# ethz-asl/reinmav-gym

Hardware: AMD Instinct MI355X
Metric: env-steps/sec (batched quadrotor3d-v0) (higher is better)
Workload: dtype f32; 1 GPU; BASELINE configs[1] (C2): quadrotor3d-v0, 65536 envs/GPU, random actions in-kernel, auto-reset; 1 step = 1 fused 64-env-step rollout launch, trajectory written to a ring of 6 buffer sets; config_id=C2, kind=quad3d, actions=random, envs_per_gpu=65536, envs_total=65536, env_steps_per_launch_per_env=64, mode=rollout, trajectory_layout=soa, trajectory_ring=6, tune=, parallelism=single GPU, finished_episodes=189717026, gathered_envs_with_a_finished_episode=65536

## Files before the change

### reinmav-gym_amd/csrc/rmav_abi.hip

```cpp
#include <cmath>
#include <cstdarg>
#include <cstdio>
#include <cstdint>
#include <cstdlib>
#include <cstring>
#include <ctime>
#include <new>

#include "rmav_handle.hpp"
#include "rmav_core_kernels.hpp"

using namespace rmav;

namespace {

thread_local char g_err[768] = "";

}

int rmav_fail(int code, const char *fmt, ...) {
    va_list ap;
    va_start(ap, fmt);
    vsnprintf(g_err, sizeof(g_err), fmt, ap);
    va_end(ap);
// ... 147 lines not shown
constexpr int64_t kEnvsPerCuSlot = 16384;
constexpr bool kSliceByDefault = false;

template <int K, int MODE, int ST>
int launch_rollout_kms(rmav_handle h, const RolloutArgs &a_in) {
    RolloutArgs a = a_in;
    take_armed_exchange(h, a, 64, publishes_start(MODE));
    const KindParams<K> kp = kind_params<K>(h);
    static_assert(!is_policy(MODE), "the policy-in-kernel rollouts are launched from rmav_policy_abi.hip");
    const size_t lds = (ST == ST_AOS_LDS) ? sizeof(float) * AosTile<Dims<K>::NS>::WORDS * (block_size(h) / 64) : 0;
    if constexpr (is_split(MODE)) {
        constexpr size_t lds_per_pair = sizeof(float) * split_words_per_pair<K, MODE>();
        const int forced = h->tune[RMAV_TUNE_SPLIT_GROUP];
        constexpr int g_max = split_pairs_max<K, MODE>();
        const int64_t count = a.slice_count ? (int64_t)a.slice_count : h->n;
        constexpr bool latency_bound = (K == QUAD2D || K == QUAD2D_SL) || MODE == ACT_CONTROLLER_SPLIT;
        const bool one_pair = latency_bound && (count <= 98304 || K == QUAD2D);
        int g = (forced >= 1 && forced <= g_max) ? forced : one_pair ? 1 : (int)((count + kEnvsPerCuSlot - 1) / kEnvsPerCuSlot);
        if (g < 1) g = 1;
        if (g > g_max) g = g_max;
        const int64_t per_wg = 64 * g;
        if (!(a.flags & F_AOS) && (int64_t)a.n_steps * Dims<K>::NS * a.pitch < ((int64_t)1 << 30)) a.flags |= F_LEAN;
        const dim3 grid((unsigned)((count + per_wg - 1) / per_wg)), block(128 * g);
        bool launched = false;
        if constexpr (ST == ST_WRITE_THROUGH) {
            if ((a.flags & (F_AOS | F_TRACK | F_AUTO_RESET)) == (F_TRACK | F_AUTO_RESET)) {
                hipLaunchKernelGGL((k_rollout<K, MODE, ST, true>), grid, block, lds_per_pair * g, h->stream, a, kp.p, kp.pc);
                launched = true;
            }
        }
        if (!launched) hipLaunchKernelGGL((k_rollout<K, MODE, ST>), grid, block, lds_per_pair * g, h->stream, a, kp.p, kp.pc);
    } else if (h->range_mask) {
        if constexpr (K != REINMAV && (MODE == ACT_BUFFER || MODE == ACT_RANDOM || MODE == ACT_CONTROLLER)) {
            if (int rc = rmav_launch_ranged_rollout(h, MODE, ST, a)) return rc;
        } else {
            return rmav_fail(RMAV_ERR_INVALID, "no ranged kernel for action mode %d", MODE);
        }
    } else {
        if (h->time_limit > 0) {
            if constexpr (K != REINMAV && (MODE == ACT_BUFFER || MODE == ACT_RANDOM || MODE == ACT_CONTROLLER)) {
                const int64_t count = a.slice_count ? (int64_t)a.slice_count : h->n;
                const dim3 grid((unsigned)((count + block_size(h) - 1) / block_size(h)));
                hipLaunchKernelGGL((k_rollout_tl<K, MODE, ST>), grid, dim3(block_size(h)), lds, h->stream, a, kp.p, kp.pc, tl_args(h));
            } else {
                return rmav_fail(RMAV_ERR_INVALID, "no time-limited kernel for action mode %d", MODE);
            }
        } else {
            hipLaunchKernelGGL((k_rollout<K, MODE, ST>), grid_for(h), dim3(block_size(h)), lds, h->stream, a, kp.p, kp.pc);
        }
    }
    return check_rollout_launch(h, a);
}

bool use_split(rmav_handle h, const RolloutArgs &a, int action_mode, int *slices, bool random_actions) {
// ... 1051 lines not shown
```

### reinmav-gym_amd/csrc/rmav_kernels.hpp

```cpp
#pragma once

#include "rmav_math.hpp"
#include "rmav_policy.hpp"
#include "rmav_policy_mfma.hpp"
#include "rmav_policy_mfma32.hpp"

namespace rmav {

enum : int { ACT_BUFFER = 0, ACT_RANDOM = 1, ACT_CONTROLLER = 2, ACT_POLICY = 3, ACT_POLICY_BF16 = 4,
              ACT_RANDOM_SPLIT = 5, ACT_CONTROLLER_SPLIT = 6,
              ACT_BUFFER_CTRL = 7,
              ACT_POLICY_F32M = 8,
              ACT_BUFFER_SPLIT = 9,
              ACT_POLICY_F16 = 10,
              ACT_POLICY_F16_SHARED = 11 };
constexpr bool is_mfma_policy(int mode) { return mode == ACT_POLICY_BF16 || mode == ACT_POLICY_F32M; }
constexpr bool is_policy(int mode) { return mode == ACT_POLICY || is_mfma_policy(mode); }
constexpr bool is_split(int mode) { return mode == ACT_RANDOM_SPLIT || mode == ACT_CONTROLLER_SPLIT || mode == ACT_BUFFER_SPLIT; }
constexpr bool split_feeds_actions(int mode) { return mode == ACT_RANDOM_SPLIT; }
constexpr bool split_self_fetch(int mode) { return mode == ACT_BUFFER_SPLIT; }
constexpr bool is_buffer(int mode) { return mode == ACT_BUFFER || mode == ACT_BUFFER_CTRL; }
constexpr bool publishes_start(int mode) { return mode != ACT_CONTROLLER_SPLIT; }
#ifndef RMAV_SPLIT_CHUNK
#define RMAV_SPLIT_CHUNK 1
// ... 205 lines not shown
#endif
typedef uint32_t u32x4_t __attribute__((ext_vector_type(4)));
template <int AUX>
__device__ __forceinline__ void buf_st4_aux(rsrc_t r, uint32_t voff, uint32_t soff, float4 v) {
    u32x4_t d;
    d[0] = __builtin_bit_cast(uint32_t, v.x);
    d[1] = __builtin_bit_cast(uint32_t, v.y);
    d[2] = __builtin_bit_cast(uint32_t, v.z);
    d[3] = __builtin_bit_cast(uint32_t, v.w);
    __builtin_amdgcn_raw_buffer_store_b128(d, r, voff, soff, AUX);
}
template <int AUX, int C>
__device__ __forceinline__ void wide_cols(const float *tile, rsrc_t r, uint32_t wave_off, uint32_t col, uint32_t lane) {
    const uint32_t cg = lane >> 4, eq = lane & 15u;
#pragma unroll
    for (int j = 0; 4 * j < C; ++j) {
        if (4 * j + 3 < C || 4 * j + (int)cg < C) {
            const float4 v = *reinterpret_cast<const float4 *>(tile + (4 * j + cg) * 64u + 4u * eq);
            buf_st4_aux<AUX>(r, wave_off + 16u * eq + cg * col, (uint32_t)(4 * j) * col, v);
        }
    }
}

template <int K, int MODE, int ST = ST_DEFAULT, bool FIXED = false>
__global__ __launch_bounds__((rollout_threads_max<K, MODE>())) void k_rollout(const RolloutArgs a, const typename Env<K>::P p_shared,
                                                    const ParamsT<double> pc_shared) {
    constexpr bool TL = false, BOOT = false, NORM = false, DR = false;
    [[maybe_unused]] const RangeArgs dr{};
    [[maybe_unused]] const ActRuleArgs ar{};
    [[maybe_unused]] const TimeLimitArgs tl{};
    [[maybe_unused]] const BootArgs bt{};
    [[maybe_unused]] const NormArgs nm{};
#include "rmav_rollout_body.inc"
}
template <int K, int MODE, int ST = ST_DEFAULT>
__global__ __launch_bounds__((rollout_threads_max<K, MODE>())) void k_rollout_tl(const RolloutArgs a, const typename Env<K>::P p_shared,
                                                       const ParamsT<double> pc_shared, const TimeLimitArgs tl) {
    constexpr bool TL = true, FIXED = false, BOOT = false, NORM = false, DR = false;
    [[maybe_unused]] const RangeArgs dr{};
    [[maybe_unused]] const ActRuleArgs ar{};
    [[maybe_unused]] const BootArgs bt{};
    [[maybe_unused]] const NormArgs nm{};
    static_assert(!is_split(MODE) && K != REINMAV, "time-limited launches run the one-wavefront kernels");
#include "rmav_rollout_body.inc"
}
template <int K, int MODE, int ST = ST_DEFAULT>
__global__ __launch_bounds__((rollout_threads_max<K, MODE>())) void k_rollout_boot(const RolloutArgs a, const typename Env<K>::P p_shared,
                                                         const ParamsT<double> pc_shared, const TimeLimitArgs tl, const BootArgs bt) {
    constexpr bool TL = true, FIXED = false, BOOT = true, NORM = false, DR = false;
    [[maybe_unused]] const RangeArgs dr{};
    [[maybe_unused]] const ActRuleArgs ar{};
    [[maybe_unused]] const NormArgs nm{};
    static_assert(MODE == ACT_POLICY_F32M && K != REINMAV, "the one-wavefront actor of time-limited handles");
#include "rmav_rollout_body.inc"
}
template <int K, bool BOOT>
__global__ __launch_bounds__((rollout_threads_max<K, ACT_POLICY_F32M>())) void k_rollout_nrm(const RolloutArgs a, const typename Env<K>::P p_shared,
// ... 398 lines not shown
```

### reinmav-gym_amd/csrc/rmav_rollout_body.inc

```
    constexpr int NS = Dims<K>::NS, NA = Dims<K>::NA;
    constexpr int AUX = StoreAux<ST>::value;
    constexpr bool SPLIT = is_split(MODE), DRAWS = split_feeds_actions(MODE);
    [[maybe_unused]] constexpr int CH = SplitTile<NS, NA, DRAWS>::CH;
    const uint32_t split_g = SPLIT ? (blockDim.x >> 7) : 1u;
    const bool upper_half = SPLIT && (uint32_t)__builtin_amdgcn_readfirstlane(threadIdx.x >> 6) >= split_g;
    const bool split_helper = upper_half;
    const uint32_t split_local = threadIdx.x - (upper_half ? 64u * split_g : 0u);
    const uint32_t gi = a.slice_first + (SPLIT ? blockIdx.x * (64u * split_g) + split_local : blockIdx.x * blockDim.x + threadIdx.x);
    const uint32_t slice_end = a.slice_count ? a.slice_first + a.slice_count : (uint32_t)a.n;
    [[maybe_unused]] float *lds_p = lds_w;
    if constexpr (SPLIT)
        lds_p = lds_w + (uint32_t)__builtin_amdgcn_readfirstlane(split_local >> 6) * SplitTile<NS, NA, DRAWS>::WORDS;
    const int64_t n = a.n;
    constexpr bool HALF = (MODE == ACT_POLICY_F32M);
    const uint32_t ge = HALF ? ((gi >> 6) << 5) + (gi & 31u) : gi;
    const bool valid = ge < slice_end;
    const uint32_t li = ((is_mfma_policy(MODE) || SPLIT) && !valid) ? slice_end - 1u : ge;
    const uint32_t col = (uint32_t)n * 4u;
    const int64_t tn = a.pitch;
    const uint32_t tcol = (uint32_t)tn * 4u;
    const uint32_t off = li * 4u;
    const bool aos = !FIXED && (a.flags & F_AOS) != 0;
    const bool track = FIXED || (a.flags & F_TRACK) != 0;
    const bool auto_reset = FIXED || (a.flags & F_AUTO_RESET) != 0;

    if constexpr (is_split(MODE)) {
        if (a.n_steps <= 0) return;
    }

    if constexpr (publishes_start(MODE)) {
        if (a.xsend && blockIdx.x == 0 && threadIdx.x == 0)
            __hip_atomic_store(a.xstarted, a.xseq, __ATOMIC_RELAXED, __HIP_MEMORY_SCOPE_AGENT);
    }

    unsigned int fin_n = 0, fin_len = 0;
    float fin_ret = 0.0f;

    if constexpr (SPLIT) {
        using ST_ = SplitTile<NS, NA, DRAWS>;
        if (!split_helper && (K == QUAD2D || K == QUAD2D_SL || split_g >= 6u)) __builtin_amdgcn_s_setprio(1);
        if (split_helper) {
            const uint64_t env_id = a.env_base + (uint64_t)li;
            const uint32_t lane = threadIdx.x & 63u;
            const int32_t T = a.n_steps;
            const int32_t nc = (T + CH - 1) / CH;
            const uint32_t wave_first = __builtin_amdgcn_readfirstlane(gi - lane);
            const int64_t end64 = a.slice_count ? (int64_t)a.slice_first + (int64_t)a.slice_count : n;
            const uint32_t n_here = (uint64_t)wave_first + 64u <= (uint64_t)end64 ? 64u
                                    : ((uint64_t)wave_first < (uint64_t)end64 ? (uint32_t)(end64 - wave_first) : 0u);
            const uint32_t aos_bytes = n_here * (uint32_t)(NS * 4);
            [[maybe_unused]] const bool wide = !aos && n_here == 64u && (tn & 3) == 0 &&
                                               (reinterpret_cast<uintptr_t>(a.done_out) & 3u) == 0;
            uint32_t aos_rd[NS];
#pragma unroll
            for (int q = 0; q < NS; ++q) {
                const uint32_t e = 64u * q + lane;
                aos_rd[q] = (e / NS) * ST_::OBS_STRIDE + (e % NS);
            }
            [[maybe_unused]] float er_m = 0.0f;
            [[maybe_unused]] int32_t el_m = 0;
            if constexpr (split_self_fetch(MODE)) {
                if (track) {
                    er_m = buf_ld(make_rsrc(a.ep_ret), off, 0);
                    el_m = (int32_t)(ep_clock0(a) - rec_ld_word(make_rsrc(a.rec), li, 2));
                    asm volatile("" : "+v"(er_m), "+v"(el_m));
                }
            }
            static_assert(!(RMAV_WIDE_DRAIN && split_self_fetch(MODE)), "the wide drain does not carry the episode statistics");
            auto episode_end = [&](float rw, float dn) {
                if constexpr (split_self_fetch(MODE)) {
                    if (track) {
                        er_m += rw;
                        el_m += 1;
                        if (dn != 0.0f) {
                            buf_st(make_rsrc(a.last_ret), off, 0, er_m);
                            rec_st_last_len(make_rsrc(a.rec), li, el_m);
                            er_m = 0.0f;
                            el_m = 0;
                        }
                    }
                }
            };
            auto fill = [&](int32_t c) {
                float *buf = lds_p + (c & 1) * ST_::A_HALF + lane;
#pragma unroll
                for (int j = 0; j < CH; ++j) {
                    const int32_t k = c * CH + j;
                    if (k < T) {
                        float act[NA];
                        random_action<K>(a.seed, env_id, a.t0 + (uint64_t)k, a.act_lo, a.act_hi, act);
#pragma unroll
                        for (int q = 0; q < NA; ++q) buf[(j * NA + q) * 64] = act[q];
                        if (a.act_out) {
                            float *dst_step = a.act_out + (int64_t)k * NA * tn;
                            if (aos) {
                                float *dst = dst_step + (int64_t)li * NA;
#pragma unroll
                                for (int q = 0; q < NA; ++q) dst[q] = act[q];
                            } else if (RMAV_WIDE_DRAIN && wide) {
                                wide_cols<AUX, NA>(buf - lane + j * NA * 64, make_rsrc(dst_step), wave_first * 4u, tcol, lane);
                            } else {
                                const rsrc_t ra = make_rsrc(dst_step);
#pragma unroll
                                for (int q = 0; q < NA; ++q) buf_st_aux<AUX>(ra, off, (uint32_t)q * tcol, act[q]);
                            }
                        }
                    }
                }
            };
            auto drain = [&](int32_t c) {
                const float *buf = lds_p + ST_::A_WORDS + (c & 1) * ST_::O_HALF + lane;
                if (RMAV_WIDE_DRAIN && wide) {
                    const float *tile = buf - lane;
// ... 55 lines not shown
                            if (aos) {
                                const float *tile = row - lane;
                                const rsrc_t ro = make_rsrc_bounded(dst_step + (int64_t)wave_first * NS, aos_bytes);
#pragma unroll
                                for (int q = 0; q < NS; ++q) o[q] = tile[aos_rd[q]];
#pragma unroll
                                for (int q = 0; q < NS; ++q) buf_st_aux<AUX>(ro, lane * 4u + 256u * q, 0u, o[q]);
                            } else {
                                const rsrc_t ro = make_rsrc(dst_step);
#pragma unroll
                                for (int q = 0; q < NS; ++q) o[q] = row[q * 64];
#pragma unroll
                                for (int q = 0; q < NS; ++q) buf_st_aux<AUX>(ro, off, (uint32_t)q * tcol, o[q]);
                            }
                        }
                        if (a.rew_out) buf_st_aux<AUX>(make_rsrc(a.rew_out + (int64_t)k * tn), off, 0, row[ST_::REW]);
                        if (a.done_out)
                            __builtin_amdgcn_raw_buffer_store_b8((uint8_t)(row[ST_::DONE] != 0.0f ? 1 : 0),
                                                                 make_rsrc(a.done_out + (int64_t)k * tn), li, 0, 0);
                        episode_end(row[ST_::REW], row[ST_::DONE]);
                    }
                }
            };
            if ((a.flags & F_LEAN) != 0) {
                static_assert(CH == 1, "one env-step per hand-over");
                constexpr int NQ = NS > NA ? NS : NA;
                uint32_t voff[NQ];
#pragma unroll
                for (int q = 0; q < NQ; ++q) voff[q] = off + (uint32_t)q * tcol;
                const rsrc_t rA = a.act_out ? make_rsrc(a.act_out) : make_rsrc_bounded(a.state, 0u);
                const rsrc_t rO = a.obs_out ? make_rsrc(a.obs_out) : make_rsrc_bounded(a.state, 0u);
                const rsrc_t rR = a.rew_out ? make_rsrc(a.rew_out) : make_rsrc_bounded(a.state, 0u);
                const rsrc_t rD = a.done_out ? make_rsrc(a.done_out) : make_rsrc_bounded(a.state, 0u);
                const uint32_t sA = (uint32_t)NA * tcol, sO = (uint32_t)NS * tcol, sR = tcol, sD = (uint32_t)tn;
                auto drain_l = [&](int32_t k) {
                    const float *row = lds_p + ST_::A_WORDS + (k & 1) * ST_::O_HALF + lane;
                    float o[NS];
#pragma unroll
                    for (int q = 0; q < NS; ++q) o[q] = row[q * 64];
                    const float rw = row[ST_::REW], dn = row[ST_::DONE];
                    if constexpr (!DRAWS) {
                        float av[NA];
#pragma unroll
                        for (int q = 0; q < NA; ++q) av[q] = row[ST_::ACT + q * 64];
#pragma unroll
                        for (int q = 0; q < NA; ++q) buf_st_aux<AUX>(rA, voff[q], (uint32_t)k * sA, av[q]);
                    }
#pragma unroll
                    for (int q = 0; q < NS; ++q) buf_st_aux<AUX>(rO, voff[q], (uint32_t)k * sO, o[q]);
                    buf_st_aux<AUX>(rR, off, (uint32_t)k * sR, rw);
                    __builtin_amdgcn_raw_buffer_store_b8((uint8_t)(dn != 0.0f ? 1 : 0), rD, li, (uint32_t)k * sD, 0);
                    episode_end(rw, dn);
                };
                {
                    [[maybe_unused]] uint32_t blk[4] = {0u, 0u, 0u, 0u};
                    [[maybe_unused]] bool blk_valid = false;
                    auto fill_l = [&](int32_t k) {
                        float *buf = lds_p + (k & 1) * ST_::A_HALF + lane;
                        float act[NA];
                        const uint64_t t = a.t0 + (uint64_t)k;
                        if constexpr (action_pairs<K>()) {
                            if ((t & 1u) == 0 || !blk_valid) {
                                random_block<K>(a.seed, env_id, t, blk);
                                blk_valid = true;
                            }
                            action_from_block<K>(blk, t, a.act_lo, a.act_hi, act);
                        } else {
                            random_action<K>(a.seed, env_id, t, a.act_lo, a.act_hi, act);
                        }
#pragma unroll
                        for (int q = 0; q < NA; ++q) buf[q * 64] = act[q];
#pragma unroll
                        for (int q = 0; q < NA; ++q) buf_st_aux<AUX>(rA, voff[q], (uint32_t)k * sA, act[q]);
                    };
                    if constexpr (DRAWS) {
                        fill_l(0);
                        if (nc >= 2) fill_l(1);
                    }
                    __syncthreads();
                    if constexpr (DRAWS) __syncthreads();
                    if (nc >= 2) {
                        if constexpr (DRAWS) {
                            if (nc >= 3) fill_l(2);
                        }
                        __syncthreads();
                    }
                    int32_t c = 2;
                    if constexpr (DRAWS && action_pairs<K>()) {
                        auto fill_half = [&](int32_t k, const uint32_t (&b)[4], uint32_t odd) {
                            float *buf = lds_p + (k & 1) * ST_::A_HALF + lane;
                            float act[NA];
                            action_from_block<K>(b, (uint64_t)odd, a.act_lo, a.act_hi, act);
#pragma unroll
                            for (int q = 0; q < NA; ++q) buf[q * 64] = act[q];
#pragma unroll
                            for (int q = 0; q < NA; ++q) buf_st_aux<AUX>(rA, voff[q], (uint32_t)k * sA, act[q]);
                        };
                        if (c + 1 < nc && ((a.t0 + (uint64_t)(c + 1)) & 1u) != 0) {
                            fill_l(c + 1);
                            drain_l(c - 2);
                            __syncthreads();
                            ++c;
                        }
                        for (; c + 2 < nc; c += 2) {
                            uint32_t b2[4];
                            random_block<K>(a.seed, env_id, a.t0 + (uint64_t)(c + 1), b2);
                            fill_half(c + 1, b2, 0u);
                            drain_l(c - 2);
                            __syncthreads();
                            fill_half(c + 2, b2, 1u);
                            drain_l(c - 1);
                            __syncthreads();
                        }
                        blk_valid = false;
                    }
                    for (; c + 1 < nc; ++c) {
                        if constexpr (DRAWS) fill_l(c + 1);
                        drain_l(c - 2);
                        __syncthreads();
                    }
                    if (nc >= 3) {
                        drain_l(nc - 3);
                        __syncthreads();
                    }
                }
                if (nc >= 2) drain_l(nc - 2);
                __syncthreads();
                drain_l(nc - 1);
                return;
            }
            {
                if constexpr (DRAWS) {
                    fill(0);
                    if (nc >= 2) fill(1);
                }
                __syncthreads();
                if constexpr (DRAWS) __syncthreads();
                for (int32_t c = 1; c < nc; ++c) {
                    if constexpr (DRAWS) {
                        if (c + 1 < nc) fill(c + 1);
                    }
// ... 2 lines not shown
                }
            }
            if (nc >= 2) drain(nc - 2);
            __syncthreads();
            drain(nc - 1);
            return;
        }
    }

    if constexpr (is_policy(MODE)) {
        constexpr int NW4 = (MODE == ACT_POLICY ? PolicyLayout<NS>::TOTAL : MODE == ACT_POLICY_F32M ? Mfma32Layout::TOTAL : MfmaLayout::TOTAL) / 4;
        const float4 *src = reinterpret_cast<const float4 *>(a.policy_w);
        float4 *dst = reinterpret_cast<float4 *>(lds_w);
        for (int q = threadIdx.x; q < NW4; q += blockDim.x) dst[q] = src[q];
        if constexpr (NORM) stage_norm(lds_w + Mfma32Layout::TOTAL, nm.tab);
        __syncthreads();
        if constexpr (MODE == ACT_POLICY_BF16) {
            scale_biases_for_tanh();
            __syncthreads();
        }
    }

    if (li < slice_end) {
        const rsrc_t r_state = make_rsrc(a.state);
        float s[NS];
#pragma unroll
        for (int c = 0; c < NS; ++c) s[c] = buf_ld(r_state, off, (uint32_t)c * col);
        float er = 0.0f;
        int32_t el = 0;
        const rsrc_t r_rec = make_rsrc(a.rec);
        int32_t sb;
        uint32_t rc;
        constexpr bool REC_WORDS = is_policy(MODE);
        if (track) er = buf_ld(make_rsrc(a.ep_ret), off, 0);
        if constexpr (REC_WORDS) {
            sb = (int32_t)rec_ld_word(r_rec, li, 0);
            rc = rec_ld_word(r_rec, li, 1);
            if (TL || track) el = (int32_t)(ep_clock0(a) - rec_ld_word(r_rec, li, 2));
        } else if (TL || track) {
            const u32x3_t q = rec_ld3(r_rec, li);
            sb = (int32_t)q.x;
            rc = q.y;
            el = (int32_t)(ep_clock0(a) - q.z);
        } else {
            const u32x2_t q = rec_ld2(r_rec, li);
            sb = (int32_t)q.x;
            rc = q.y;
        }
        const uint64_t env_id = a.env_base + (uint64_t)li;
        typename Env<K>::P pl = p_shared;
        ParamsT<double> pcl = pc_shared;
        if constexpr (K != REINMAV) {
            if (a.pe[0] || a.pe[1] || a.pe[2]) {
                const double m = a.pe[0] ? (double)a.pe[0][li] : (double)pc_shared.mass;
                const double ml = a.pe[1] ? (double)a.pe[1][li] : (double)pc_shared.load_mass;
                const double L = a.pe[2] ? (double)a.pe[2][li] : (double)pc_shared.L;
                override_params(pl, m, ml, L);
                override_params(pcl, m, ml, L);
            }
        }
        const typename Env<K>::P &p = pl;
        const ParamsT<double> &pc = pcl;
        double tenv = 0.0;
        if constexpr (K == REINMAV) tenv = a.env_time[li];

        constexpr bool SPARE_LDS = spare_in_lds<K, MODE>();
        [[maybe_unused]] float spare[SPARE_LDS ? 1 : NS];
        [[maybe_unused]] float *lds_spare = nullptr;
        if constexpr (SPARE_LDS)
            lds_spare = lds_w + split_g * SplitTile<NS, NA, DRAWS>::WORDS +
                        (uint32_t)__builtin_amdgcn_readfirstlane(split_local >> 6) * SplitTile<NS, NA, DRAWS>::SPARE + (threadIdx.x & 63u);
        bool have_spare = false;
        [[maybe_unused]] float spare_pe[3];
        if constexpr (DR) spare_pe[0] = spare_pe[1] = spare_pe[2] = 0.0f;
        if (K != REINMAV && auto_reset && a.n_steps >= 8) {
            if constexpr (SPARE_LDS) {
                float sp[NS];
                reset_state<K>(a.seed, env_id, rc, sp);
#pragma unroll
                for (int c = 0; c < NS; ++c) lds_spare[c * 64] = sp[c];
            } else {
                reset_state<K>(a.seed, env_id, rc, spare);
            }
            if constexpr (DR) range_draw(dr, a.seed, env_id, rc, spare_pe);
            have_spare = true;
        }

        [[maybe_unused]] float *tile = nullptr;
        [[maybe_unused]] uint32_t tile_rd[NS];
        [[maybe_unused]] bool full_wave = false;
        [[maybe_unused]] uint32_t wave_obs_base = 0;
        if constexpr (ST == ST_AOS_LDS) {
            const uint32_t lane = threadIdx.x & 63u;
            const uint32_t wave_first = __builtin_amdgcn_readfirstlane(gi - lane);
            tile = lds_w + __builtin_amdgcn_readfirstlane(threadIdx.x >> 6) * AosTile<NS>::WORDS;
            full_wave = wave_first + 64u <= slice_end;
            wave_obs_base = wave_first * (uint32_t)(NS * 4);
#pragma unroll
            for (int j = 0; j < NS; ++j) {
                const uint32_t e = 64u * j + lane;
                tile_rd[j] = (e / NS) * AosTile<NS>::STRIDE + (e % NS);
            }
        }

        const float *act_in = a.act_in;
        float *act_out = (!is_buffer(MODE) && !SPLIT) ? a.act_out : nullptr;
        float *obs_out = a.obs_out;
// ... 15 lines not shown
            }
            pol_logp0 = -sl - 0.5f * (float)NA * 1.8378770664093453f;
        }

        float act_pre[NA];
        auto load_actions = [&](const float *src_step, float (&dst)[NA]) {
            if (aos) {
                const float *src = src_step + (int64_t)li * NA;
#pragma unroll
                for (int c = 0; c < NA; ++c) dst[c] = src[c];
            } else {
                const rsrc_t r = make_rsrc(src_step);
#pragma unroll
                for (int c = 0; c < NA; ++c) dst[c] = buf_ld(r, off, (uint32_t)c * tcol);
            }
        };
        if constexpr (is_buffer(MODE)) load_actions(act_in, act_pre);
        [[maybe_unused]] float ring_pre[split_self_fetch(MODE) ? buf_prefetch<NA>() : 1][NA];
        [[maybe_unused]] float *lds_ring = nullptr;
        [[maybe_unused]] auto ring_fetch = [&](int32_t k0) {
            if constexpr (split_self_fetch(MODE)) {
#pragma unroll
                for (int d = 0; d < buf_prefetch<NA>(); ++d)
                    if (k0 + d < a.n_steps) load_actions(a.act_in + (int64_t)(k0 + d) * NA * tn, ring_pre[d]);
            }
        };
        [[maybe_unused]] auto ring_put = [&]() {
            if constexpr (split_self_fetch(MODE)) {
#pragma unroll
                for (int d = 0; d < buf_prefetch<NA>(); ++d)
#pragma unroll
                    for (int c = 0; c < NA; ++c) lds_ring[(d * NA + c) * 64] = ring_pre[d][c];
            }
        };
        if constexpr (split_self_fetch(MODE)) {
            using STB = SplitTile<NS, NA, DRAWS>;
            lds_ring = lds_w + split_g * (STB::WORDS + (spare_in_lds<K, MODE>() ? STB::SPARE : 0)) +
                       (uint32_t)__builtin_amdgcn_readfirstlane(split_local >> 6) * buf_ring_words<NA>() + (threadIdx.x & 63u);
            ring_fetch(0);
            ring_put();
            ring_fetch(buf_prefetch<NA>());
        }
        [[maybe_unused]] float act_nx[NA];
        if constexpr (split_feeds_actions(MODE)) {
            static_assert(CH == 1, "one env-step per hand-over");
            __syncthreads();
            const float *buf = lds_p + (threadIdx.x & 63u);
#pragma unroll
            for (int c = 0; c < NA; ++c) act_nx[c] = buf[c * 64];
            __syncthreads();
        }

        for (int32_t k = 0; k < a.n_steps; ++k) {
            float act[NA];
            if constexpr (is_mfma_policy(MODE)) {
                float x[16], mean[4], val0, z[4];
                if constexpr (NORM) {
                    norm_state16<NS>(lds_w + Mfma32Layout::TOTAL, s, x);
                } else {
#pragma unroll
                    for (int c = 0; c < 16; ++c) x[c] = (c < NS) ? s[c] : 0.0f;
                }
                if constexpr (MODE == ACT_POLICY_BF16) policy_forward_mfma(x, mean, val0);
                else policy_forward_mfma32<NS>(x, mean, val0);
                gaussian4(a.seed, env_id, a.t0 + (uint64_t)k, z);
                float q = 0.0f;
#pragma unroll
                for (int c = 0; c < NA; ++c) {
                    act[c] = rfma(pol_std[c], z[c], mean[c]);
                    q = rfma(z[c], z[c], q);
                }
                if constexpr (NORM) q *= ar.noise;
                buf_st(make_rsrc(logp_out), off, 0, rfma(-0.5f, q, pol_logp0));
                buf_st(make_rsrc(val_out), off, 0, val0);
                logp_out += n;
                val_out += n;
            } else if constexpr (MODE == ACT_POLICY) {
                using PL = PolicyLayout<NS>;
                XVec<PL::NSP> x;
#pragma unroll
                for (int c = 0; c < PL::NSP; ++c) x.v[c] = (c < NS) ? s[c] : 0.0f;
                const float4 m4 = mlp_forward<NS>(x, 0u);
                const float4 v4 = mlp_forward<NS>(x, (uint32_t)PL::NET);
                const float mean[4] = {m4.x, m4.y, m4.z, m4.w};
                const float val[1] = {v4.x};
                float z[4];
                gaussian4(a.seed, env_id, a.t0 + (uint64_t)k, z);
                float q = 0.0f;
#pragma unroll
                for (int c = 0; c < NA; ++c) {
                    act[c] = rfma(pol_std[c], z[c], mean[c]);
                    q = rfma(z[c], z[c], q);
                }
                buf_st(make_rsrc(logp_out), off, 0, rfma(-0.5f, q, pol_logp0));
                buf_st(make_rsrc(val_out), off, 0, val[0]);
                logp_out += n;
                val_out += n;
            } else if constexpr (is_buffer(MODE)) {
#pragma unroll
                for (int c = 0; c < NA; ++c) act[c] = act_pre[c];
                act_in += (int64_t)NA * tn;
                if (k + 1 < a.n_steps) load_actions(act_in, act_pre);
            } else if constexpr (MODE == ACT_RANDOM) {
                random_action<K>(a.seed, env_id, a.t0 + (uint64_t)k, a.act_lo, a.act_hi, act);
            } else if constexpr (split_feeds_actions(MODE)) {
#pragma unroll
                for (int c = 0; c < NA; ++c) act[c] = act_nx[c];
                const float *buf = lds_p + ((k + 1) & 1) * SplitTile<NS, NA, true>::A_HALF + (threadIdx.x & 63u);
#pragma unroll
                for (int c = 0; c < NA; ++c) act_nx[c] = buf[c * 64];
            } else if constexpr (MODE == ACT_CONTROLLER_SPLIT) {
                if ((k % CH) == 0) __syncthreads();
                env_control<K>(s, pc, act);
            } else if constexpr (split_self_fetch(MODE)) {
                if ((k % CH) == 0) __syncthreads();
                constexpr int D = buf_prefetch<NA>();
                static_assert((D & (D - 1)) == 0, "burst length: a power of two");
                const int32_t slot = k & (D - 1);
                if (slot == 0 && k > 0) {
                    ring_put();
                    ring_fetch(k + D);
                }
                const float *rb = lds_ring + slot * (NA * 64);
#pragma unroll
                for (int c = 0; c < NA; ++c) act[c] = rb[c * 64];
            } else if constexpr (K == REINMAV) {
#pragma unroll
// ... 76 lines not shown
                }
                if (__ballot(done) != 0) {
                    if constexpr (TL) {
                        if (done && !track) el = 0;
                    }
                    if (track && done) {
                        if constexpr (!split_self_fetch(MODE)) {
                            buf_st(make_rsrc(a.last_ret), off, 0, er);
                            rec_st_last_len(make_rsrc(a.rec), li, el);
                        }
                        if (valid && !(HALF && (threadIdx.x & 32u))) {
                            fin_n += 1;
                            fin_len += (unsigned int)el;
                            fin_ret += er;
                        }
                        er = 0.0f;
                        el = 0;
                    }
                    if (K != REINMAV && auto_reset) {
                        const bool rst = done;
                        if (__ballot(rst && !have_spare) != 0) {
                            if (!have_spare) {
                                float sp[NS];
                                reset_state<K>(a.seed, env_id, rc, sp);
#pragma unroll
                                for (int c = 0; c < NS; ++c) {
                                    if constexpr (SPARE_LDS) lds_spare[c * 64] = sp[c];
                                    else spare[c] = sp[c];
                                }
                                if constexpr (DR) range_draw(dr, a.seed, env_id, rc, spare_pe);
                                have_spare = true;
                            }
                        }
                        if (rst) {
#pragma unroll
                            for (int c = 0; c < NS; ++c) {
                                if constexpr (SPARE_LDS) s[c] = lds_spare[c * 64];
                                else s[c] = spare[c];
                            }
                            if constexpr (DR) range_apply(dr, a.pe, pc_shared, li, off, spare_pe, pl, pcl);
                            have_spare = false;
                            rc += 1;
                        }
                    }
                }
            } else {
                if (track) {
                    er += r;
                    el += 1;
                    if (done) {
                        buf_st(make_rsrc(a.last_ret), off, 0, er);
                        rec_st_last_len(make_rsrc(a.rec), li, el);
                        if (valid && !(HALF && (threadIdx.x & 32u))) {
                            fin_n += 1;
                            fin_len += (unsigned int)el;
                            fin_ret += er;
                        }
                        er = 0.0f;
                        el = 0;
                    }
                } else if (TL) {
                    el += 1;
                    if (done) el = 0;
                }
                if (K != REINMAV && auto_reset) {
                    const bool rst = done;
                    if (__ballot(rst && !have_spare) != 0) {
                        if (!have_spare) {
                            float sp[NS];
                            reset_state<K>(a.seed, env_id, rc, sp);
#pragma unroll
                            for (int c = 0; c < NS; ++c) {
                                if constexpr (SPARE_LDS) lds_spare[c * 64] = sp[c];
                                else spare[c] = sp[c];
                            }
                            if constexpr (DR) range_draw(dr, a.seed, env_id, rc, spare_pe);
                            have_spare = true;
                        }
                    }
                    if (rst) {
#pragma unroll
                        for (int c = 0; c < NS; ++c) {
                            if constexpr (SPARE_LDS) s[c] = lds_spare[c * 64];
                            else s[c] = spare[c];
                        }
                        if constexpr (DR) range_apply(dr, a.pe, pc_shared, li, off, spare_pe, pl, pcl);
                        have_spare = false;
                        rc += 1;
                    }
                }
            }
            if constexpr (SPLIT) {
                using ST_ = SplitTile<NS, NA, DRAWS>;
                float *row = lds_p + ST_::A_WORDS + ((k / CH) & 1) * ST_::O_HALF + (k % CH) * ST_::O_ROW +
                             (threadIdx.x & 63u);
                {
                    if (aos) {
                        float *mine = row + (threadIdx.x & 63u) * (ST_::OBS_STRIDE - 1);
#pragma unroll
                        for (int c = 0; c < NS; ++c) mine[c] = s[c];
                    } else {
#pragma unroll
                        for (int c = 0; c < NS; ++c) row[c * 64] = s[c];
                    }
                }
                row[ST_::REW] = r;
                row[ST_::DONE] = done ? 1.0f : 0.0f;
                if constexpr (!DRAWS) {
#pragma unroll
                    for (int c = 0; c < NA; ++c) row[ST_::ACT + c * 64] = act[c];
                }
                if constexpr (split_feeds_actions(MODE)) __syncthreads();
            } else if (obs_out) {
                if (ST == ST_AOS_LDS && full_wave) {
                    __builtin_amdgcn_fence(__ATOMIC_RELEASE, "wavefront");
                    __builtin_amdgcn_wave_barrier();
                    float *row = tile + (threadIdx.x & 63u) * AosTile<NS>::STRIDE;
#pragma unroll
                    for (int c = 0; c < NS; ++c) row[c] = s[c];
                    __builtin_amdgcn_fence(__ATOMIC_RELEASE, "wavefront");
                    __builtin_amdgcn_wave_barrier();
                    __builtin_amdgcn_fence(__ATOMIC_ACQUIRE, "wavefront");
                    const rsrc_t ro = make_rsrc(obs_out);
                    const uint32_t voff = (threadIdx.x & 63u) * 4u;
#pragma unroll
                    for (int j = 0; j < NS; ++j) buf_st_aux<AUX>(ro, voff, wave_obs_base + 256u * j, tile[tile_rd[j]]);
                } else if (aos) {
                    float *dst = obs_out + (int64_t)li * NS;
#pragma unroll
                    for (int c = 0; c < NS; ++c) dst[c] = s[c];
                } else {
                    const rsrc_t ro = make_rsrc(obs_out);
#pragma unroll
                    for (int c = 0; c < NS; ++c) buf_st_aux<AUX>(ro, off, (uint32_t)c * tcol, s[c]);
                }
// ... 30 lines not shown
            const float4 v4 = mlp_forward<NS>(x, (uint32_t)PL::NET);
            buf_st(make_rsrc(val_out), off, 0, v4.x);
        }
#pragma unroll
        for (int c = 0; c < NS; ++c) buf_st(r_state, off, (uint32_t)c * col, s[c]);
        if constexpr (MODE == ACT_BUFFER_CTRL && K != REINMAV) {
            float a2[NA];
            env_control<K>(s, pc, a2);
            if (aos) {
                float *dst = a.ctrl_out + (int64_t)li * NA;
#pragma unroll
                for (int c = 0; c < NA; ++c) dst[c] = a2[c];
            } else {
                const rsrc_t rc2 = make_rsrc(a.ctrl_out);
#pragma unroll
                for (int c = 0; c < NA; ++c) buf_st(rc2, off, (uint32_t)c * col, a2[c]);
            }
        }
        if constexpr (K == REINMAV) a.env_time[li] = tenv;
        if (track) buf_st(make_rsrc(a.ep_ret), off, 0, er);
        if constexpr (is_policy(MODE)) {
            rec_st_word(make_rsrc(a.rec), li, 0, (uint32_t)sb);
            rec_st_word(make_rsrc(a.rec), li, 1, rc);
            if (TL || track) rec_st_word(make_rsrc(a.rec), li, 2, ep_clock0(a) + (uint32_t)a.n_steps - (uint32_t)el);
        } else if (TL || track) {
            rec_st3(make_rsrc(a.rec), li, u32x3_t{(uint32_t)sb, rc, ep_clock0(a) + (uint32_t)a.n_steps - (uint32_t)el});
        } else {
            rec_st2(make_rsrc(a.rec), li, u32x2_t{(uint32_t)sb, rc});
        }
    }

    if (track) {
        Totals *slot = a.totals + (gi >> 6);
        if (a.n_steps == 1) {
            if (fin_n != 0) {
                atomicAdd(&slot->episodes, (unsigned long long)fin_n);
                atomicAdd(&slot->length_sum, (unsigned long long)fin_len);
                atomicAdd(&slot->return_sum, (double)fin_ret);
            }
        } else if (__ballot(fin_n != 0) != 0) {
            const unsigned int wn = is_mfma_policy(MODE) ? wave_sum_x(fin_n) : wave_sum(fin_n);
            const unsigned int wl = is_mfma_policy(MODE) ? wave_sum_x(fin_len) : wave_sum(fin_len);
            const float wr = is_mfma_policy(MODE) ? wave_sum_x(fin_ret) : wave_sum(fin_ret);
            if ((threadIdx.x & 63) == 0) {
                atomicAdd(&slot->episodes, (unsigned long long)wn);
                atomicAdd(&slot->length_sum, (unsigned long long)wl);
                atomicAdd(&slot->return_sum, (double)wr);
            }
        }
    }

    if (a.xsend) {
        asm volatile("s_waitcnt vmcnt(0)" ::: "memory");
        if (valid && !(HALF && (threadIdx.x & 32u))) {
            const float lr = a.last_ret[li];
            const int32_t ll = a.rec[li].last_len;
            __hip_atomic_store(a.xsend + li, __builtin_bit_cast(int32_t, lr), __ATOMIC_RELAXED, __HIP_MEMORY_SCOPE_AGENT);
// ... 7 lines not shown
```

Before: 103.9 billion env-steps/s.

## Pass hot rollout scalars as leading kernel args and reorder split-kernel prologue

For the random-action split rollout kernel, the frequently used scalars (state pointer, seed, env base, t0, n, block size, step count, flags, slice) are passed as separate leading kernel arguments. They are read from those instead of the RolloutArgs struct, which is meant to shorten the kernarg loads in the kernel head. The start-publish atomic moves after the state load, and the spare reset-state draw is deferred until after the first step's hand-over barrier so it is off the critical startup path. In the helper wave, the drain of old trajectory rows is issued before the fill of the next actions so stores overlap better. This adds a second kernel overload and macro plumbing, and changes the timing of the xstarted publish.

Measured after the change: 99.85 billion env-steps/s. -3.9%, worse.

```diff
diff --git a/reinmav-gym_amd/csrc/rmav_abi.hip b/reinmav-gym_amd/csrc/rmav_abi.hip
--- a/reinmav-gym_amd/csrc/rmav_abi.hip
+++ b/reinmav-gym_amd/csrc/rmav_abi.hip
@@ -193,14 +193,26 @@
         const int64_t per_wg = 64 * g;
         if (!(a.flags & F_AOS) && (int64_t)a.n_steps * Dims<K>::NS * a.pitch < ((int64_t)1 << 30)) a.flags |= F_LEAN;
         const dim3 grid((unsigned)((count + per_wg - 1) / per_wg)), block(128 * g);
+        auto launch = [&](auto fixed) {
+            constexpr bool FX = decltype(fixed)::value;
+            if constexpr (RMAV_HEAD_A && split_feeds_actions(MODE)) {
+                using Hot = void (*)(float *, uint64_t, uint64_t, uint64_t, uint32_t, uint32_t, int32_t, uint32_t, uint32_t, uint32_t, const RolloutArgs,
+                                     const typename Env<K>::P, const ParamsT<double>);
+                hipLaunchKernelGGL(static_cast<Hot>(k_rollout<K, MODE, ST, FX>), grid, block, lds_per_pair * g, h->stream, a.state, a.seed,
+                                   a.env_base, a.t0, (uint32_t)a.n, block.x, a.n_steps, a.flags, a.slice_first, a.slice_count, a, kp.p, kp.pc);
+            } else {
+                using Plain = void (*)(const RolloutArgs, const typename Env<K>::P, const ParamsT<double>);
+                hipLaunchKernelGGL(static_cast<Plain>(k_rollout<K, MODE, ST, FX>), grid, block, lds_per_pair * g, h->stream, a, kp.p, kp.pc);
+            }
+        };
         bool launched = false;
         if constexpr (ST == ST_WRITE_THROUGH) {
             if ((a.flags & (F_AOS | F_TRACK | F_AUTO_RESET)) == (F_TRACK | F_AUTO_RESET)) {
-                hipLaunchKernelGGL((k_rollout<K, MODE, ST, true>), grid, block, lds_per_pair * g, h->stream, a, kp.p, kp.pc);
+                launch(std::true_type{});
                 launched = true;
             }
         }
-        if (!launched) hipLaunchKernelGGL((k_rollout<K, MODE, ST>), grid, block, lds_per_pair * g, h->stream, a, kp.p, kp.pc);
+        if (!launched) launch(std::false_type{});
     } else if (h->range_mask) {
         if constexpr (K != REINMAV && (MODE == ACT_BUFFER || MODE == ACT_RANDOM || MODE == ACT_CONTROLLER)) {
             if (int rc = rmav_launch_ranged_rollout(h, MODE, ST, a)) return rc;
diff --git a/reinmav-gym_amd/csrc/rmav_kernels.hpp b/reinmav-gym_amd/csrc/rmav_kernels.hpp
--- a/reinmav-gym_amd/csrc/rmav_kernels.hpp
+++ b/reinmav-gym_amd/csrc/rmav_kernels.hpp
@@ -251,6 +251,18 @@
     }
 }
 
+#ifndef RMAV_HEAD_A
+#define RMAV_HEAD_A 1
+#endif
+#ifndef RMAV_HEAD_B
+#define RMAV_HEAD_B 1
+#endif
+#ifndef RMAV_HEAD_C
+#define RMAV_HEAD_C 1
+#endif
+#define RMAV_ROLLOUT_HOT 0
+#define RMAV_HOT(f) a.f
+#define RMAV_EP_CLOCK0 ep_clock0(a)
 template <int K, int MODE, int ST = ST_DEFAULT, bool FIXED = false>
 __global__ __launch_bounds__((rollout_threads_max<K, MODE>())) void k_rollout(const RolloutArgs a, const typename Env<K>::P p_shared,
                                                     const ParamsT<double> pc_shared) {
@@ -262,6 +274,41 @@
     [[maybe_unused]] const NormArgs nm{};
 #include "rmav_rollout_body.inc"
 }
+struct RolloutHot {
+    float *state;
+    uint64_t seed, env_base, t0;
+    uint32_t n;
+    uint32_t block;
+    int32_t n_steps;
+    uint32_t flags;
+    uint32_t slice_first, slice_count;
+};
+#undef RMAV_ROLLOUT_HOT
+#undef RMAV_HOT
+#undef RMAV_EP_CLOCK0
+#define RMAV_ROLLOUT_HOT 1
+#define RMAV_HOT(f) f##_pl
+#define RMAV_EP_CLOCK0 (uint32_t)t0_pl
+template <int K, int MODE, int ST = ST_DEFAULT, bool FIXED = false>
+__global__ __launch_bounds__((rollout_threads_max<K, MODE>())) std::enable_if_t<split_feeds_actions(MODE)> k_rollout(float *state_pl, uint64_t seed_pl, uint64_t env_base_pl, uint64_t t0_pl,
+                                                    uint32_t n_pl, uint32_t block_pl, int32_t n_steps_pl, uint32_t flags_pl,
+                                                    uint32_t slice_first_pl, uint32_t slice_count_pl, const RolloutArgs a,
+                                                    const typename Env<K>::P p_shared, const ParamsT<double> pc_shared) {
+    static_assert(split_feeds_actions(MODE), "the leading-scalar form is the random-action two-wavefront kernels'");
+    constexpr bool TL = false, BOOT = false, NORM = false, DR = false;
+    [[maybe_unused]] const RangeArgs dr{};
+    [[maybe_unused]] const ActRuleArgs ar{};
+    [[maybe_unused]] const TimeLimitArgs tl{};
+    [[maybe_unused]] const BootArgs bt{};
+    [[maybe_unused]] const NormArgs nm{};
+#include "rmav_rollout_body.inc"
+}
+#undef RMAV_ROLLOUT_HOT
+#undef RMAV_HOT
+#undef RMAV_EP_CLOCK0
+#define RMAV_ROLLOUT_HOT 0
+#define RMAV_HOT(f) a.f
+#define RMAV_EP_CLOCK0 ep_clock0(a)
 template <int K, int MODE, int ST = ST_DEFAULT>
 __global__ __launch_bounds__((rollout_threads_max<K, MODE>())) void k_rollout_tl(const RolloutArgs a, const typename Env<K>::P p_shared,
                                                        const ParamsT<double> pc_shared, const TimeLimitArgs tl) {
diff --git a/reinmav-gym_amd/csrc/rmav_rollout_body.inc b/reinmav-gym_amd/csrc/rmav_rollout_body.inc
--- a/reinmav-gym_amd/csrc/rmav_rollout_body.inc
+++ b/reinmav-gym_amd/csrc/rmav_rollout_body.inc
@@ -2,16 +2,20 @@
     constexpr int AUX = StoreAux<ST>::value;
     constexpr bool SPLIT = is_split(MODE), DRAWS = split_feeds_actions(MODE);
     [[maybe_unused]] constexpr int CH = SplitTile<NS, NA, DRAWS>::CH;
+#if RMAV_ROLLOUT_HOT
+    const uint32_t split_g = block_pl >> 7;
+#else
     const uint32_t split_g = SPLIT ? (blockDim.x >> 7) : 1u;
+#endif
     const bool upper_half = SPLIT && (uint32_t)__builtin_amdgcn_readfirstlane(threadIdx.x >> 6) >= split_g;
     const bool split_helper = upper_half;
     const uint32_t split_local = threadIdx.x - (upper_half ? 64u * split_g : 0u);
-    const uint32_t gi = a.slice_first + (SPLIT ? blockIdx.x * (64u * split_g) + split_local : blockIdx.x * blockDim.x + threadIdx.x);
-    const uint32_t slice_end = a.slice_count ? a.slice_first + a.slice_count : (uint32_t)a.n;
+    const uint32_t gi = RMAV_HOT(slice_first) + (SPLIT ? blockIdx.x * (64u * split_g) + split_local : blockIdx.x * blockDim.x + threadIdx.x);
+    const uint32_t slice_end = RMAV_HOT(slice_count) ? RMAV_HOT(slice_first) + RMAV_HOT(slice_count) : (uint32_t)RMAV_HOT(n);
     [[maybe_unused]] float *lds_p = lds_w;
     if constexpr (SPLIT)
         lds_p = lds_w + (uint32_t)__builtin_amdgcn_readfirstlane(split_local >> 6) * SplitTile<NS, NA, DRAWS>::WORDS;
-    const int64_t n = a.n;
+    const int64_t n = RMAV_HOT(n);
     constexpr bool HALF = (MODE == ACT_POLICY_F32M);
     const uint32_t ge = HALF ? ((gi >> 6) << 5) + (gi & 31u) : gi;
     const bool valid = ge < slice_end;
@@ -20,18 +24,20 @@
     const int64_t tn = a.pitch;
     const uint32_t tcol = (uint32_t)tn * 4u;
     const uint32_t off = li * 4u;
-    const bool aos = !FIXED && (a.flags & F_AOS) != 0;
-    const bool track = FIXED || (a.flags & F_TRACK) != 0;
-    const bool auto_reset = FIXED || (a.flags & F_AUTO_RESET) != 0;
+    const bool aos = !FIXED && (RMAV_HOT(flags) & F_AOS) != 0;
+    const bool track = FIXED || (RMAV_HOT(flags) & F_TRACK) != 0;
+    const bool auto_reset = FIXED || (RMAV_HOT(flags) & F_AUTO_RESET) != 0;
 
     if constexpr (is_split(MODE)) {
-        if (a.n_steps <= 0) return;
+        if (RMAV_HOT(n_steps) <= 0) return;
     }
 
+#if !RMAV_ROLLOUT_HOT
     if constexpr (publishes_start(MODE)) {
         if (a.xsend && blockIdx.x == 0 && threadIdx.x == 0)
             __hip_atomic_store(a.xstarted, a.xseq, __ATOMIC_RELAXED, __HIP_MEMORY_SCOPE_AGENT);
     }
+#endif
 
     unsigned int fin_n = 0, fin_len = 0;
     float fin_ret = 0.0f;
@@ -40,12 +46,12 @@
         using ST_ = SplitTile<NS, NA, DRAWS>;
         if (!split_helper && (K == QUAD2D || K == QUAD2D_SL || split_g >= 6u)) __builtin_amdgcn_s_setprio(1);
         if (split_helper) {
-            const uint64_t env_id = a.env_base + (uint64_t)li;
+            const uint64_t env_id = RMAV_HOT(env_base) + (uint64_t)li;
             const uint32_t lane = threadIdx.x & 63u;
-            const int32_t T = a.n_steps;
+            const int32_t T = RMAV_HOT(n_steps);
             const int32_t nc = (T + CH - 1) / CH;
             const uint32_t wave_first = __builtin_amdgcn_readfirstlane(gi - lane);
-            const int64_t end64 = a.slice_count ? (int64_t)a.slice_first + (int64_t)a.slice_count : n;
+            const int64_t end64 = RMAV_HOT(slice_count) ? (int64_t)RMAV_HOT(slice_first) + (int64_t)RMAV_HOT(slice_count) : n;
             const uint32_t n_here = (uint64_t)wave_first + 64u <= (uint64_t)end64 ? 64u
                                     : ((uint64_t)wave_first < (uint64_t)end64 ? (uint32_t)(end64 - wave_first) : 0u);
             const uint32_t aos_bytes = n_here * (uint32_t)(NS * 4);
@@ -62,7 +68,7 @@
             if constexpr (split_self_fetch(MODE)) {
                 if (track) {
                     er_m = buf_ld(make_rsrc(a.ep_ret), off, 0);
-                    el_m = (int32_t)(ep_clock0(a) - rec_ld_word(make_rsrc(a.rec), li, 2));
+                    el_m = (int32_t)(RMAV_EP_CLOCK0 - rec_ld_word(make_rsrc(a.rec), li, 2));
                     asm volatile("" : "+v"(er_m), "+v"(el_m));
                 }
             }
@@ -88,7 +94,7 @@
                     const int32_t k = c * CH + j;
                     if (k < T) {
                         float act[NA];
-                        random_action<K>(a.seed, env_id, a.t0 + (uint64_t)k, a.act_lo, a.act_hi, act);
+                        random_action<K>(RMAV_HOT(seed), env_id, RMAV_HOT(t0) + (uint64_t)k, a.act_lo, a.act_hi, act);
 #pragma unroll
                         for (int q = 0; q < NA; ++q) buf[(j * NA + q) * 64] = act[q];
                         if (a.act_out) {
@@ -190,16 +196,16 @@
                     }
                 }
             };
-            if ((a.flags & F_LEAN) != 0) {
+            if ((RMAV_HOT(flags) & F_LEAN) != 0) {
                 static_assert(CH == 1, "one env-step per hand-over");
                 constexpr int NQ = NS > NA ? NS : NA;
                 uint32_t voff[NQ];
 #pragma unroll
                 for (int q = 0; q < NQ; ++q) voff[q] = off + (uint32_t)q * tcol;
-                const rsrc_t rA = a.act_out ? make_rsrc(a.act_out) : make_rsrc_bounded(a.state, 0u);
-                const rsrc_t rO = a.obs_out ? make_rsrc(a.obs_out) : make_rsrc_bounded(a.state, 0u);
-                const rsrc_t rR = a.rew_out ? make_rsrc(a.rew_out) : make_rsrc_bounded(a.state, 0u);
-                const rsrc_t rD = a.done_out ? make_rsrc(a.done_out) : make_rsrc_bounded(a.state, 0u);
+                const rsrc_t rA = a.act_out ? make_rsrc(a.act_out) : make_rsrc_bounded(RMAV_HOT(state), 0u);
+                const rsrc_t rO = a.obs_out ? make_rsrc(a.obs_out) : make_rsrc_bounded(RMAV_HOT(state), 0u);
+                const rsrc_t rR = a.rew_out ? make_rsrc(a.rew_out) : make_rsrc_bounded(RMAV_HOT(state), 0u);
+                const rsrc_t rD = a.done_out ? make_rsrc(a.done_out) : make_rsrc_bounded(RMAV_HOT(state), 0u);
                 const uint32_t sA = (uint32_t)NA * tcol, sO = (uint32_t)NS * tcol, sR = tcol, sD = (uint32_t)tn;
                 auto drain_l = [&](int32_t k) {
                     const float *row = lds_p + ST_::A_WORDS + (k & 1) * ST_::O_HALF + lane;
@@ -226,15 +232,15 @@
                     auto fill_l = [&](int32_t k) {
                         float *buf = lds_p + (k & 1) * ST_::A_HALF + lane;
                         float act[NA];
-                        const uint64_t t = a.t0 + (uint64_t)k;
+                        const uint64_t t = RMAV_HOT(t0) + (uint64_t)k;
                         if constexpr (action_pairs<K>()) {
                             if ((t & 1u) == 0 || !blk_valid) {
-                                random_block<K>(a.seed, env_id, t, blk);
+                                random_block<K>(RMAV_HOT(seed), env_id, t, blk);
                                 blk_valid = true;
                             }
                             action_from_block<K>(blk, t, a.act_lo, a.act_hi, act);
                         } else {
-                            random_action<K>(a.seed, env_id, t, a.act_lo, a.act_hi, act);
+                            random_action<K>(RMAV_HOT(seed), env_id, t, a.act_lo, a.act_hi, act);
                         }
 #pragma unroll
                         for (int q = 0; q < NA; ++q) buf[q * 64] = act[q];
@@ -264,27 +270,31 @@
 #pragma unroll
                             for (int q = 0; q < NA; ++q) buf_st_aux<AUX>(rA, voff[q], (uint32_t)k * sA, act[q]);
                         };
-                        if (c + 1 < nc && ((a.t0 + (uint64_t)(c + 1)) & 1u) != 0) {
+                        if (c + 1 < nc && ((RMAV_HOT(t0) + (uint64_t)(c + 1)) & 1u) != 0) {
+                            if constexpr (RMAV_HEAD_C) drain_l(c - 2);
                             fill_l(c + 1);
-                            drain_l(c - 2);
+                            if constexpr (!RMAV_HEAD_C) drain_l(c - 2);
                             __syncthreads();
                             ++c;
                         }
                         for (; c + 2 < nc; c += 2) {
                             uint32_t b2[4];
-                            random_block<K>(a.seed, env_id, a.t0 + (uint64_t)(c + 1), b2);
+                            random_block<K>(RMAV_HOT(seed), env_id, RMAV_HOT(t0) + (uint64_t)(c + 1), b2);
+                            if constexpr (RMAV_HEAD_C) drain_l(c - 2);
                             fill_half(c + 1, b2, 0u);
-                            drain_l(c - 2);
+                            if constexpr (!RMAV_HEAD_C) drain_l(c - 2);
                             __syncthreads();
+                            if constexpr (RMAV_HEAD_C) drain_l(c - 1);
                             fill_half(c + 2, b2, 1u);
-                            drain_l(c - 1);
+                            if constexpr (!RMAV_HEAD_C) drain_l(c - 1);
                             __syncthreads();
                         }
                         blk_valid = false;
                     }
                     for (; c + 1 < nc; ++c) {
+                        if constexpr (RMAV_HEAD_C) drain_l(c - 2);
                         if constexpr (DRAWS) fill_l(c + 1);
-                        drain_l(c - 2);
+                        if constexpr (!RMAV_HEAD_C) drain_l(c - 2);
                         __syncthreads();
                     }
                     if (nc >= 3) {
@@ -333,10 +343,14 @@
     }
 
     if (li < slice_end) {
-        const rsrc_t r_state = make_rsrc(a.state);
+        const rsrc_t r_state = make_rsrc(RMAV_HOT(state));
         float s[NS];
 #pragma unroll
         for (int c = 0; c < NS; ++c) s[c] = buf_ld(r_state, off, (uint32_t)c * col);
+#if RMAV_ROLLOUT_HOT
+        if (a.xsend && blockIdx.x == 0 && threadIdx.x == 0)
+            __hip_atomic_store(a.xstarted, a.xseq, __ATOMIC_RELAXED, __HIP_MEMORY_SCOPE_AGENT);
+#endif
         float er = 0.0f;
         int32_t el = 0;
         const rsrc_t r_rec = make_rsrc(a.rec);
@@ -347,18 +361,18 @@
         if constexpr (REC_WORDS) {
             sb = (int32_t)rec_ld_word(r_rec, li, 0);
             rc = rec_ld_word(r_rec, li, 1);
-            if (TL || track) el = (int32_t)(ep_clock0(a) - rec_ld_word(r_rec, li, 2));
+            if (TL || track) el = (int32_t)(RMAV_EP_CLOCK0 - rec_ld_word(r_rec, li, 2));
         } else if (TL || track) {
             const u32x3_t q = rec_ld3(r_rec, li);
             sb = (int32_t)q.x;
             rc = q.y;
-            el = (int32_t)(ep_clock0(a) - q.z);
+            el = (int32_t)(RMAV_EP_CLOCK0 - q.z);
         } else {
             const u32x2_t q = rec_ld2(r_rec, li);
             sb = (int32_t)q.x;
             rc = q.y;
         }
-        const uint64_t env_id = a.env_base + (uint64_t)li;
+        const uint64_t env_id = RMAV_HOT(env_base) + (uint64_t)li;
         typename Env<K>::P pl = p_shared;
         ParamsT<double> pcl = pc_shared;
         if constexpr (K != REINMAV) {
@@ -384,16 +398,17 @@
         bool have_spare = false;
         [[maybe_unused]] float spare_pe[3];
         if constexpr (DR) spare_pe[0] = spare_pe[1] = spare_pe[2] = 0.0f;
-        if (K != REINMAV && auto_reset && a.n_steps >= 8) {
+        constexpr bool LATE_SPARE = RMAV_HEAD_B && split_feeds_actions(MODE) && !DR;
+        if (!LATE_SPARE && K != REINMAV && auto_reset && RMAV_HOT(n_steps) >= 8) {
             if constexpr (SPARE_LDS) {
                 float sp[NS];
-                reset_state<K>(a.seed, env_id, rc, sp);
+                reset_state<K>(RMAV_HOT(seed), env_id, rc, sp);
 #pragma unroll
                 for (int c = 0; c < NS; ++c) lds_spare[c * 64] = sp[c];
             } else {
-                reset_state<K>(a.seed, env_id, rc, spare);
-            }
-            if constexpr (DR) range_draw(dr, a.seed, env_id, rc, spare_pe);
+                reset_state<K>(RMAV_HOT(seed), env_id, rc, spare);
+            }
+            if constexpr (DR) range_draw(dr, RMAV_HOT(seed), env_id, rc, spare_pe);
             have_spare = true;
         }
 
@@ -455,7 +470,7 @@
             if constexpr (split_self_fetch(MODE)) {
 #pragma unroll
                 for (int d = 0; d < buf_prefetch<NA>(); ++d)
-                    if (k0 + d < a.n_steps) load_actions(a.act_in + (int64_t)(k0 + d) * NA * tn, ring_pre[d]);
+                    if (k0 + d < RMAV_HOT(n_steps)) load_actions(a.act_in + (int64_t)(k0 + d) * NA * tn, ring_pre[d]);
             }
         };
         [[maybe_unused]] auto ring_put = [&]() {
@@ -484,7 +499,7 @@
             __syncthreads();
         }
 
-        for (int32_t k = 0; k < a.n_steps; ++k) {
+        for (int32_t k = 0; k < RMAV_HOT(n_steps); ++k) {
             float act[NA];
             if constexpr (is_mfma_policy(MODE)) {
                 float x[16], mean[4], val0, z[4];
@@ -496,7 +511,7 @@
                 }
                 if constexpr (MODE == ACT_POLICY_BF16) policy_forward_mfma(x, mean, val0);
                 else policy_forward_mfma32<NS>(x, mean, val0);
-                gaussian4(a.seed, env_id, a.t0 + (uint64_t)k, z);
+                gaussian4(RMAV_HOT(seed), env_id, RMAV_HOT(t0) + (uint64_t)k, z);
                 float q = 0.0f;
 #pragma unroll
                 for (int c = 0; c < NA; ++c) {
@@ -518,7 +533,7 @@
                 const float mean[4] = {m4.x, m4.y, m4.z, m4.w};
                 const float val[1] = {v4.x};
                 float z[4];
-                gaussian4(a.seed, env_id, a.t0 + (uint64_t)k, z);
+                gaussian4(RMAV_HOT(seed), env_id, RMAV_HOT(t0) + (uint64_t)k, z);
                 float q = 0.0f;
 #pragma unroll
                 for (int c = 0; c < NA; ++c) {
@@ -533,9 +548,9 @@
 #pragma unroll
                 for (int c = 0; c < NA; ++c) act[c] = act_pre[c];
                 act_in += (int64_t)NA * tn;
-                if (k + 1 < a.n_steps) load_actions(act_in, act_pre);
+                if (k + 1 < RMAV_HOT(n_steps)) load_actions(act_in, act_pre);
             } else if constexpr (MODE == ACT_RANDOM) {
-                random_action<K>(a.seed, env_id, a.t0 + (uint64_t)k, a.act_lo, a.act_hi, act);
+                random_action<K>(RMAV_HOT(seed), env_id, RMAV_HOT(t0) + (uint64_t)k, a.act_lo, a.act_hi, act);
             } else if constexpr (split_feeds_actions(MODE)) {
 #pragma unroll
                 for (int c = 0; c < NA; ++c) act[c] = act_nx[c];
@@ -658,13 +673,13 @@
                         if (__ballot(rst && !have_spare) != 0) {
                             if (!have_spare) {
                                 float sp[NS];
-                                reset_state<K>(a.seed, env_id, rc, sp);
+                                reset_state<K>(RMAV_HOT(seed), env_id, rc, sp);
 #pragma unroll
                                 for (int c = 0; c < NS; ++c) {
                                     if constexpr (SPARE_LDS) lds_spare[c * 64] = sp[c];
                                     else spare[c] = sp[c];
                                 }
-                                if constexpr (DR) range_draw(dr, a.seed, env_id, rc, spare_pe);
+                                if constexpr (DR) range_draw(dr, RMAV_HOT(seed), env_id, rc, spare_pe);
                                 have_spare = true;
                             }
                         }
@@ -704,13 +719,13 @@
                     if (__ballot(rst && !have_spare) != 0) {
                         if (!have_spare) {
                             float sp[NS];
-                            reset_state<K>(a.seed, env_id, rc, sp);
+                            reset_state<K>(RMAV_HOT(seed), env_id, rc, sp);
 #pragma unroll
                             for (int c = 0; c < NS; ++c) {
                                 if constexpr (SPARE_LDS) lds_spare[c * 64] = sp[c];
                                 else spare[c] = sp[c];
                             }
-                            if constexpr (DR) range_draw(dr, a.seed, env_id, rc, spare_pe);
+                            if constexpr (DR) range_draw(dr, RMAV_HOT(seed), env_id, rc, spare_pe);
                             have_spare = true;
                         }
                     }
@@ -747,6 +762,20 @@
                     for (int c = 0; c < NA; ++c) row[ST_::ACT + c * 64] = act[c];
                 }
                 if constexpr (split_feeds_actions(MODE)) __syncthreads();
+                if constexpr (LATE_SPARE) {
+                    if (k == 0 && auto_reset && RMAV_HOT(n_steps) >= 8 && __ballot(!have_spare) != 0) {
+                        if (!have_spare) {
+                            float sp[NS];
+                            reset_state<K>(RMAV_HOT(seed), env_id, rc, sp);
+#pragma unroll
+                            for (int c = 0; c < NS; ++c) {
+                                if constexpr (SPARE_LDS) lds_spare[c * 64] = sp[c];
+                                else spare[c] = sp[c];
+                            }
+                            have_spare = true;
+                        }
+                    }
+                }
             } else if (obs_out) {
                 if (ST == ST_AOS_LDS && full_wave) {
                     __builtin_amdgcn_fence(__ATOMIC_RELEASE, "wavefront");
@@ -823,9 +852,9 @@
         if constexpr (is_policy(MODE)) {
             rec_st_word(make_rsrc(a.rec), li, 0, (uint32_t)sb);
             rec_st_word(make_rsrc(a.rec), li, 1, rc);
-            if (TL || track) rec_st_word(make_rsrc(a.rec), li, 2, ep_clock0(a) + (uint32_t)a.n_steps - (uint32_t)el);
+            if (TL || track) rec_st_word(make_rsrc(a.rec), li, 2, RMAV_EP_CLOCK0 + (uint32_t)RMAV_HOT(n_steps) - (uint32_t)el);
         } else if (TL || track) {
-            rec_st3(make_rsrc(a.rec), li, u32x3_t{(uint32_t)sb, rc, ep_clock0(a) + (uint32_t)a.n_steps - (uint32_t)el});
+            rec_st3(make_rsrc(a.rec), li, u32x3_t{(uint32_t)sb, rc, RMAV_EP_CLOCK0 + (uint32_t)RMAV_HOT(n_steps) - (uint32_t)el});
         } else {
             rec_st2(make_rsrc(a.rec), li, u32x2_t{(uint32_t)sb, rc});
         }
@@ -833,7 +862,7 @@
 
     if (track) {
         Totals *slot = a.totals + (gi >> 6);
-        if (a.n_steps == 1) {
+        if (RMAV_HOT(n_steps) == 1) {
             if (fin_n != 0) {
                 atomicAdd(&slot->episodes, (unsigned long long)fin_n);
                 atomicAdd(&slot->length_sum, (unsigned long long)fin_len);
```
